# allenai/satlas-super-resolution

Hardware: AMD Instinct MI355X
Metric: G+D train-step images/sec (higher is better)
Workload: dtype fp32h

## Files before the change

satlas_super_resolution_amd/csrc/conv_x3r.hip:

```cpp
#include "conv_x3r_core.h"

#ifdef SSR_PROBE
#define RPROBE(cond, k) do { if (cond) g_probe[(blockIdx.y * gridDim.x + blockIdx.x) * 16 + (k)] = __builtin_amdgcn_s_memtime(); } while (0)
#else
#define RPROBE(cond, k)
#endif

namespace {

template <int NTW, int NU, int EP, int TH = 8, int AM = 0>
__global__ __launch_bounds__((XrT<NTW, NU, TH>::NTHR)) void conv_x3r_kernel(const ssr_conv_desc d) {
    constexpr bool EX = AM == 1, H = AM == 2;
    using T = XrT<NTW, NU, TH>;
    constexpr int NT = NTW, NTT = T::NTT, NMF = T::NMF, BN = T::BN, WR = T::WR, MT = T::MT;
    constexpr int G_NPIX = T::NPIX, G_SUB = T::SUB, G_PV = T::PV, G_NPV = T::NPV;
    extern __shared__ __attribute__((aligned(16))) char smem[];
    int* ctl = reinterpret_cast<int*>(smem + T::CTL);
    const int ctl_addr = (int)(size_t)(__attribute__((address_space(3))) char*)(smem + T::CTL);
    const int tid = threadIdx.x, lane = tid & 63, wave = __builtin_amdgcn_readfirstlane(tid >> 6);
    const int tiles_x = (d.Gw + 15) / 16, tiles_y = (d.Gh + TH - 1) / TH;
    int b = blockIdx.x;
    const int tx_i = b % tiles_x; b /= tiles_x;
    const int ty_i = b % tiles_y;
    const int n = b / tiles_y;
    const int gy0 = ty_i * TH, gx0 = tx_i * 16;
    const int co0 = blockIdx.y * BN;
    const int Cin = d.Cin, Cin2 = d.Cin2;
    const int nchunks = (Cin + Cin2 + 15) / 16;
    const int cout_pad = d.CoutPad;
    const int tapstride = cout_pad * 64, wchunk = 9 * tapstride;
    RPROBE(tid == 0, 0);
    if (tid < 4 + NMF) ctl[tid] = 0;
    __syncthreads();

    f32x16 acc[MT][NT];
#pragma unroll
    for (int t = 0; t < MT; ++t)
#pragma unroll
        for (int u = 0; u < NT; ++u)
#pragma unroll
            for (int r = 0; r < 16; ++r) acc[t][u][r] = 0.f;

    if (wave >= NMF) {
        const int pw = wave - NMF;
        const int pt = tid - 64 * NMF;
#ifdef XR_PRIO
        __builtin_amdgcn_s_setprio(3);
#endif
        const int part = pt & 3, p4 = pt >> 2;
        int ppix[G_NPV];
#pragma unroll
        for (int q = 0; q < G_NPV; ++q) {
            const int pix = p4 + 64 * q;
            const int py = pix / XR_PW, px = pix - py * XR_PW;
            const int ly = gy0 + py - d.pad_y, lx = gx0 + px - d.pad_x;
            const bool okp = pix < G_NPIX && ly >= 0 && ly < d.Hi && lx >= 0 && lx < d.Wi;
            ppix[q] = okp ? (n * d.Hi + ly) * d.Wi + lx : -1;
        }
        const int plo0 = p4 * XR_ROWB + part * 8;
        const long xbytes = (long)d.N * d.Hi * d.Wi * 4;
        const void* xp = d.x.p;
        const void* x2p = d.x2.p ? d.x2.p : d.x.p;
        const int x_cs = d.x.cs, x_coff = d.x.coff, x2_cs = d.x2.p ? d.x2.cs : d.x.cs, x2_coff = d.x2.p ? d.x2.coff : d.x.coff;
        u32x4 rq[XR_PQ][G_NPV];
        auto load_chunk = [&](int c, auto jc) {
            constexpr int j = decltype(jc)::value;
            const bool live = c < nchunks;
            const int c0 = c * 16;
            const bool in_x = c0 < Cin;
            const int cb = in_x ? c0 : c0 - Cin, clim = live ? (in_x ? Cin : Cin2) : 0;
            const int cs = in_x ? x_cs : x2_cs, coff = in_x ? x_coff : x2_coff;
            const __amdgpu_buffer_rsrc_t rs = xr_rsrc(in_x ? xp : x2p, xbytes * cs);
            const int k = cb + part * 4;
#pragma unroll
            for (int q = 0; q < G_NPV; ++q) {
                const int off = (ppix[q] * cs + coff + k) * 4;
                const bool okl = (k < clim) & (ppix[q] >= 0);
#ifdef XR_X_NOXLOAD
                rq[j][q] = u32x4{(unsigned)off, (unsigned)okl, 0u, 0u};
#else
                rq[j][q] = __builtin_amdgcn_raw_buffer_load_b128(rs, okl ? off : XR_OOB, 0, 0);
#endif
            }
        };
        static_for<0, XR_PQ>([&](auto jc) { __builtin_amdgcn_sched_barrier(0); load_chunk(decltype(jc)::value, jc); __builtin_amdgcn_sched_barrier(0); });
        RPROBE(pt == 0, 8);
        int cfree = XR_NS;
        for (int c0 = 0; c0 < nchunks; c0 += XR_PQ) {
            static_for<0, XR_PQ>([&](auto jc) {
                constexpr int j = decltype(jc)::value;
                const int c = c0 + j;
                if (c < nchunks) {
                    if (c >= cfree) {
                        int spin = 0;
                        for (; spin < XR_SPIN_MAX; ++spin) {
                            cfree = xr_minN<NMF>(ctl_addr + 16) + XR_NS;
                            if (c < cfree) break;
                            __builtin_amdgcn_s_sleep(2);
                        }
                        if (spin == XR_SPIN_MAX) __builtin_trap();
                    }
                    char* base = smem + (c % XR_NS) * G_SUB;
#pragma unroll
                    for (int q = 0; q < G_NPV; ++q) {
#ifdef XR_X_NOSTORE
                        asm volatile("" :: "v"(rq[j][q]));
                        continue;
#endif
                        if constexpr (EX) {
                            if (q < G_NPV - 1 || pt < G_PV - (G_NPV - 1) * 256)
                                *reinterpret_cast<u32x4*>(base + p4 * XR_ROWB + part * 16 + q * 64 * XR_ROWB) = rq[j][q];
                        } else {
                            uint2 hi, lo;
                            split_f32x4<H>(rq[j][q], hi, lo);
                            if (q < G_NPV - 1 || pt < G_PV - (G_NPV - 1) * 256) {
                                *reinterpret_cast<uint2*>(base + plo0 + q * 64 * XR_ROWB) = hi;
                                *reinterpret_cast<uint2*>(base + plo0 + q * 64 * XR_ROWB + 32) = lo;
                            }
                        }
                    }
                    asm volatile("" ::: "memory");
                    if (lane == 0) *(xr_lds_int)(uintptr_t)(ctl_addr + 4 * pw) = c + 1;
                    asm volatile("" ::: "memory");
#if defined(XR_PRIO) && XR_PRIO == 1
                    if (c == 0) __builtin_amdgcn_s_setprio(0);
#endif
                }
                __builtin_amdgcn_sched_barrier(0);
                load_chunk(c + XR_PQ, jc);
                __builtin_amdgcn_sched_barrier(0);
            });
        }
        RPROBE(pt == 0, 9);
    } else {
        const int w = wave & 3, ug = wave >> 2;
        const int i = lane & 31, gq = lane >> 5;
        const int a_lane = ((i >> 4) * XR_PW + epi_col<XR_ROT>(i)) * XR_ROWB + gq * 16;
        const __amdgpu_buffer_rsrc_t rsw = xr_rsrc(d.w, (long)nchunks * wchunk);
        const int w_lane = (co0 + 32 * NTW * ug + i) * 64 + gq * 16;
        const int nitems = 3 * nchunks;
        const int nj = nitems > w ? (nitems - w + 3) / 4 : 0;
        const int glast = w + 4 * (nj - 1);
        if (nj == 0) {
            if (lane == 0) *(xr_lds_int)(uintptr_t)(ctl_addr + 16 + 4 * wave) = 0x3fffffff;
        } else {
            bf16x8 wf[WR][NT][2];
            constexpr int TPS = T::TPS, SPT = T::SPT, NSUB = 3 * SPT, NSETS = T::NSETS, PD = NSETS - 1;
            bf16x8 af[NSETS][TPS][2];
            auto load_w = [&](int g_, auto kxc, auto sc) {
                constexpr int kx = decltype(kxc)::value, s = decltype(sc)::value;
                const int gg = g_ < glast ? g_ : glast;
                const int c = gg / 3, ky = gg - 3 * c;
                const int off = c * wchunk + (ky * 3 + kx) * tapstride + w_lane;
#pragma unroll
                for (int u = 0; u < NT; ++u) {
                    wf[s][u][0] = __builtin_bit_cast(bf16x8, __builtin_amdgcn_raw_buffer_load_b128(rsw, off + u * 2048, 0, 0));
                    wf[s][u][1] = __builtin_bit_cast(bf16x8, __builtin_amdgcn_raw_buffer_load_b128(rsw, off + u * 2048 + 32, 0, 0));
                }
            };
            auto issue_a = [&](int base, auto qc, auto sc, auto hc) {
                constexpr int q = decltype(qc)::value, kx = q / SPT, part = q % SPT, s = decltype(sc)::value, H = decltype(hc)::value;
#pragma unroll
                for (int t2 = 0; t2 < TPS; ++t2)
                    af[s][t2][H] = *reinterpret_cast<const bf16x8*>(smem + base + kx * XR_ROWB + (part * TPS + t2) * XR_TILEB + 32 * H);
            };
            int avail = 0;
            auto ensure = [&](int c) {
                if (avail > c) return;
                int spin = 0;
                for (; spin < XR_SPIN_MAX; ++spin) {
                    avail = xr_min4(ctl_addr);
                    if (avail > c) break;
                    __builtin_amdgcn_s_sleep(1);
                }
                if (spin == XR_SPIN_MAX) __builtin_trap();
            };
            auto base_of = [&](int g_) { const int c = g_ / 3, ky = g_ - 3 * c; return (c % XR_NS) * G_SUB + ky * XR_PW * XR_ROWB + a_lane; };
            using I0 = std::integral_constant<int, 0>;
            using I1 = std::integral_constant<int, 1>;
#ifndef XR_WPRE
#define XR_WPRE 99
#endif
            constexpr int WPRE = XR_WPRE < WR ? XR_WPRE : WR;
            static_for<0, WPRE>([&](auto sc) {
                constexpr int s = decltype(sc)::value;
                __builtin_amdgcn_sched_barrier(0);
                load_w(w + 4 * (s / 3), std::integral_constant<int, s % 3>{}, sc);
                __builtin_amdgcn_sched_barrier(0);
            });
            RPROBE(tid == 0, 1);
            int g = w, c_cur = g / 3;
            int base_cur = base_of(g);
            ensure(c_cur);
            static_for<WPRE, WR>([&](auto sc) {
                constexpr int s = decltype(sc)::value;
                __builtin_amdgcn_sched_barrier(0);
                load_w(w + 4 * (s / 3), std::integral_constant<int, s % 3>{}, sc);
                __builtin_amdgcn_sched_barrier(0);
            });
            RPROBE(tid == 0, 2);
            static_for<0, PD>([&](auto qc) {
                issue_a(base_cur, qc, std::integral_constant<int, decltype(qc)::value % NSETS>{}, I1{});
                issue_a(base_cur, qc, std::integral_constant<int, decltype(qc)::value % NSETS>{}, I0{});
            });
            int gn = g + 4 < glast ? g + 4 : glast;
            int c_next = gn / 3, base_next = base_of(gn);
            int gnn = gn, c_nn = c_next, base_nn = base_next;
            auto body = [&](int j, auto jpc) {
                constexpr int JP = decltype(jpc)::value;
                static_for<0, NSUB>([&](auto qc) {
                    constexpr int q = decltype(qc)::value, kx = q / SPT, part = q % SPT, qn = q + PD;
                    constexpr int ws = (JP * 3 + kx) % WR, as = (JP * NSUB + q) % NSETS, asn = (JP * NSUB + qn) % NSETS;
                    auto group = [&](auto pc) {
                        constexpr int P = decltype(pc)::value;
                        if constexpr (EX) {
                            constexpr int H = P == 0 ? 1 : 0, S0 = P == 2 ? 2 : 0, S1 = P == 1 ? 2 : 4;
#pragma unroll
                            for (int sidx = S0; sidx < S1; ++sidx)
#pragma unroll
                                for (int t2 = 0; t2 < TPS; ++t2)
#pragma unroll
                                    for (int u = 0; u < NT; ++u) {
                                        const f32x4 av = __builtin_bit_cast(f32x4, af[as][t2][H]), bv = __builtin_bit_cast(f32x4, wf[ws][u][H]);
                                        acc[part * TPS + t2][u] = __builtin_amdgcn_mfma_f32_32x32x2f32(av[sidx], bv[sidx], acc[part * TPS + t2][u], 0, 0, 0);
                                    }
                        } else {
#pragma unroll
                            for (int t2 = 0; t2 < TPS; ++t2)
#pragma unroll
                                for (int u = 0; u < NT; ++u)
                                    acc[part * TPS + t2][u] = split_mfma<H>(af[as][t2][P == 0 ? 1 : 0], wf[ws][u][P == 1 ? 1 : 0], acc[part * TPS + t2][u]);
                        }
                    };
                    auto reads = [&](auto hc) {
#ifndef XR_X_NOA
                        if constexpr (qn < NSUB) issue_a(base_cur, std::integral_constant<int, qn>{}, std::integral_constant<int, asn>{}, hc);
                        else issue_a(base_next, std::integral_constant<int, qn - NSUB>{}, std::integral_constant<int, asn>{}, hc);
#endif
                    };
                    __builtin_amdgcn_sched_barrier(0);
                    if constexpr (qn == NSUB) {
                        if (c_next > c_cur) {
                            asm volatile("" ::: "memory");
                            if (lane == 0) *(xr_lds_int)(uintptr_t)(ctl_addr + 16 + 4 * wave) = c_next;
                            asm volatile("" ::: "memory");
                        }
                        ensure(c_next);
                        __builtin_amdgcn_sched_barrier(0);
                    }
                    group(std::integral_constant<int, 0>{});
                    __builtin_amdgcn_sched_barrier(0);
                    reads(I1{});
                    if constexpr (part == 0) {
#ifndef XR_X_NOW
                        constexpr int wsp = (JP * 3 + kx + WR - 1) % WR, ioff = (kx + WR - 1) / 3, tap = (kx + WR - 1) % 3;
                        load_w(g + 4 * ioff, std::integral_constant<int, tap>{}, std::integral_constant<int, wsp>{});
#endif
                    }
                    __builtin_amdgcn_sched_barrier(0);
                    group(std::integral_constant<int, 1>{});
                    __builtin_amdgcn_sched_barrier(0);
                    reads(I0{});
                    if constexpr (q == 0) {
                        gnn = g + 8 < glast ? g + 8 : glast;
                        c_nn = gnn / 3;
                        base_nn = base_of(gnn);
                    }
                    __builtin_amdgcn_sched_barrier(0);
                    group(std::integral_constant<int, 2>{});
                    __builtin_amdgcn_sched_barrier(0);
                });
                g += 4;
                c_cur = c_next; base_cur = base_next;
                gn = gnn; c_next = c_nn; base_next = base_nn;
#ifdef SSR_PROBE
                if (j < 5) RPROBE(tid == 0, 3 + j);
#endif
            };
            if constexpr (WR == 6 || (NSUB % NSETS) != 0) {
                for (int j = 0; j < nj; j += 2) {
                    body(j, std::integral_constant<int, 0>{});
                    if (j + 1 < nj) body(j + 1, std::integral_constant<int, 1>{});
                }
            } else {
                for (int j = 0; j < nj; ++j) body(j, std::integral_constant<int, 0>{});
            }
            asm volatile("" ::: "memory");
            if (lane == 0) *(xr_lds_int)(uintptr_t)(ctl_addr + 16 + 4 * wave) = 0x3fffffff;
        }
    }
    __syncthreads();
    RPROBE(tid == 0, 10);

    const bool is_mfma = wave < NMF;
    const int me = is_mfma ? (wave & 3) : wave - NMF;
    const int ut = is_mfma ? NTW * (wave >> 2) : 1;
#ifndef XR_X_NORED
    if (is_mfma) {
#pragma unroll
        for (int t = 0; t < MT; ++t)
#pragma unroll
            for (int u = 0; u < NT; ++u)
                if (!(t == me && u == 0)) {
                    char* sp = smem + ((me * MT + t) * NTT + ut + u) * XR_SLOT + lane * 16;
#pragma unroll
                    for (int q = 0; q < 4; ++q) {
                        f32x4 v = {acc[t][u][4 * q], acc[t][u][4 * q + 1], acc[t][u][4 * q + 2], acc[t][u][4 * q + 3]};
                        *reinterpret_cast<f32x4*>(sp + q * 1024) = v;
                    }
                }
    }
#endif
    __syncthreads();
    if ((is_mfma || NTW == 2) && me < MT) {
        f32x16 own;
#pragma unroll
        for (int r = 0; r < 16; ++r) own[r] = 0.f;
        if (is_mfma) {
#pragma unroll
            for (int t = 0; t < MT; ++t)
                if (t == me) own = acc[t][0];
        }
        f32x16 sum;
#pragma unroll
        for (int s = 0; s < 4; ++s) {
            f32x16 part;
            const char* sp = smem + ((s * MT + me) * NTT + ut) * XR_SLOT + lane * 16;
#ifdef XR_X_NORED
            part = own;
            asm volatile("" : "+v"(part));
#else
#pragma unroll
            for (int q = 0; q < 4; ++q) {
                const f32x4 v = *reinterpret_cast<const f32x4*>(sp + q * 1024);
                part[4 * q] = v[0]; part[4 * q + 1] = v[1]; part[4 * q + 2] = v[2]; part[4 * q + 3] = v[3];
            }
#endif
            const bool mine = is_mfma && s == me;
#pragma unroll
            for (int r = 0; r < 16; ++r) {
                const float p = mine ? own[r] : part[r];
                sum[r] = s == 0 ? p : sum[r] + p;
            }
        }
        if constexpr (H) {
#pragma unroll
            for (int r = 0; r < 16; ++r) sum[r] *= SSR_F32H_UNSCALE;
        }
        char* slab = smem + (((is_mfma ? me : 0) * MT + me) * NTT + ut) * XR_SLOT;
        const int cb = co0 + 32 * ut;
#ifdef XR_X_NOEPI
        float keep = 0.f;
#pragma unroll
        for (int r = 0; r < 16; ++r) keep += sum[r];
        if (keep == 123.456f) reinterpret_cast<float*>(d.y.p)[tid] = keep;
#else
        if constexpr (EP == XR_EP_GENERIC) conv_epilogue<float, XR_ROT>(d, sum, cb, n, gy0 + 2 * me, gx0, lane, slab);
        else xr_epilogue<EP>(d, sum, cb, n, gy0 + 2 * me, gx0, lane, slab);
#endif
    }
    RPROBE(tid == 0, 11);
}

template <int NTW, int NU, int EP, int TH = 8, int AM = 0>
int launch_x3r(const ssr_conv_desc& d, hipStream_t st) {
    using T = XrT<NTW, NU, TH>;
    auto kern = conv_x3r_kernel<NTW, NU, EP, TH, AM>;
    static bool attr_done[SSR_MAX_DEVICES] = {};
    const int dev = ssr_device_ordinal();
    if (!attr_done[dev]) {
        hipError_t e = hipFuncSetAttribute(reinterpret_cast<const void*>(kern), hipFuncAttributeMaxDynamicSharedMemorySize, T::LDS);
        if (e != hipSuccess) return (int)e;
        attr_done[dev] = true;
    }
    const int tiles = ((d.Gw + 15) / 16) * ((d.Gh + TH - 1) / TH) * d.N;
    hipLaunchKernelGGL(kern, dim3(tiles, d.CoutPad / T::BN, 1), dim3(T::NTHR), T::LDS, st, d);
    SSR_LAUNCH_CHECK();
    return SSR_OK;
}

int xr_pick_epilogue(const ssr_conv_desc& d) {
    static const bool generic_only = [] { const char* e = getenv("SSR_X3R_EPI"); return e && e[0] == '0'; }();
    if (generic_only) return XR_EP_GENERIC;
    const long lim = 0x7fffff00L, npx = (long)d.N * d.Ho * d.Wo * 4;
    auto vok = [&](const ssr_view& v) { return (v.cs % 4) == 0 && (v.coff % 4) == 0 && ((uintptr_t)v.p % 16) == 0 && npx * v.cs <= lim; };
    if (d.fix_list || d.y0.p || d.y1.p || d.accumulate || d.m_relu || (d.Cout % 4) != 0 || !vok(d.y)) return XR_EP_GENERIC;
    if (d.oys != 1 || d.oxs != 1 || d.oyo != 0 || d.oxo != 0 || d.Ho < d.Gh || d.Wo < d.Gw) return XR_EP_GENERIC;
    const bool r1 = d.r1.p != nullptr, r2 = d.r2.p != nullptr, m = d.m.p != nullptr;
    if (d.act == SSR_ACT_LRELU && d.alpha == 1.f && !r1 && !r2 && !m) return XR_EP_LRELU;
    if (d.act == SSR_ACT_NONE && !m && (!r1 || (d.r1_nc >= d.Cout && vok(d.r1))) && (!r2 || (d.r2_nc >= d.Cout && vok(d.r2)))) return XR_EP_LIN;
    if (d.act == SSR_ACT_NONE && d.alpha == 1.f && m && !r1 && !r2 && d.m_c0 == 0 && d.m_c1 >= d.Cout && vok(d.m)) return XR_EP_MASK;
    return XR_EP_GENERIC;
}

template <int NTW, int NU, int TH = 8, int AM = 0>
int launch_x3r_ep(const ssr_conv_desc& d, hipStream_t st) {
    switch (xr_pick_epilogue(d)) {
        case XR_EP_LRELU: return launch_x3r<NTW, NU, XR_EP_LRELU, TH, AM>(d, st);
        case XR_EP_LIN: return launch_x3r<NTW, NU, XR_EP_LIN, TH, AM>(d, st);
        case XR_EP_MASK: return launch_x3r<NTW, NU, XR_EP_MASK, TH, AM>(d, st);
        default: return launch_x3r<NTW, NU, XR_EP_GENERIC, TH, AM>(d, st);
    }
}

int xr_tile_height(const ssr_conv_desc& d, int form) {
    static const int forced = [] { const char* e = getenv("SSR_X3_REGTILE_TH"); return e ? atoi(e) : 0; }();
    if (form != 0) return 8;
    if (forced == 4 || forced == 8) return forced;
    const long tiles8 = (long)((d.Gw + 15) / 16) * ((d.Gh + 7) / 8) * d.N * (d.CoutPad / 32);
    return (tiles8 <= 160 && d.Gh > 4) ? 4 : 8;
}

int xr_wide_form(const ssr_conv_desc& d) {
    static const int f = [] { const char* e = getenv("SSR_X3_REGTILE_NT2"); return !e ? 1 : e[0] == '0' ? 0 : e[0] == '8' ? 2 : 1; }();
    if ((d.CoutPad % 64) != 0) return 0;
    static const bool split_off = [] { const char* e = getenv("SSR_X3_REGTILE_SPLIT"); return e && e[0] == '0'; }();
    const long tiles = (long)((d.Gw + 15) / 16) * ((d.Gh + 7) / 8) * d.N;
    if (!split_off && tiles * (d.CoutPad / 64) <= 160) return 0;
    return (f == 2 && xr_pick_epilogue(d) == XR_EP_GENERIC) ? 1 : f;
}

}

void ssr_conv_x3r_instance(const ssr_conv_desc& d, int* ntw, int* nu, int* ep) {
    int f = xr_wide_form(d);
    if ((d.dtype == SSR_F32 || d.dtype == SSR_F32H) && f == 2) f = 1;
    *ntw = f == 1 ? 2 : 1;
    *nu = f == 2 ? 2 : 1;
    *ep = xr_pick_epilogue(d);
}
int ssr_conv_x3r_tile_height(const ssr_conv_desc& d) { return xr_tile_height(d, xr_wide_form(d)); }

bool ssr_conv_x3r_shape_ok(const ssr_conv_desc& d) {
    static const bool ex_off = [] { const char* e = getenv("SSR_F32_REGTILE"); return e && e[0] == '0'; }();
    if (!(d.dtype == SSR_F32X3 || d.dtype == SSR_F32H || (d.dtype == SSR_F32 && !ex_off)) || d.fix_list) return false;
    if (d.dtype == SSR_F32 && (d.act == SSR_ACT_RELU || d.m_relu)) return false;
    if (!(d.KH == 3 && d.KW == 3 && d.stride == 1 && d.pad_y == 1 && d.pad_x == 1 && d.up == 1 && !d.s2d)) return false;
    if (d.Gh != d.Hi || d.Gw != d.Wi || (d.CoutPad % 32) != 0) return false;
    if (d.x2.p && (d.Cin % 16) != 0) return false;
    const long lim = 0x7fffff00L, npx = (long)d.N * d.Hi * d.Wi * 4;
    if (npx * d.x.cs > lim || (d.x2.p && npx * d.x2.cs > lim)) return false;
    if ((long)((d.Cin + d.Cin2 + 15) / 16) * 9 * d.CoutPad * 64 > lim) return false;
    return true;
}

bool ssr_conv_x3r_qualifies(const ssr_conv_desc& d) {
    static const bool off = [] { const char* e = getenv("SSR_X3_REGTILE"); return e && e[0] == '0'; }();
    if (off || !ssr_conv_x3r_shape_ok(d)) return false;
    return d.Gh <= 64 && d.Gw <= 64 && d.Cin + d.Cin2 >= 16;
}

bool ssr_conv_x3r_try(const ssr_conv_desc& d, hipStream_t st, int* rc, bool force) {
    if (force ? !ssr_conv_x3r_shape_ok(d) : !ssr_conv_x3r_qualifies(d)) return false;
    const int f = xr_wide_form(d);
    if (d.dtype == SSR_F32) {
        if (f != 0) *rc = launch_x3r_ep<2, 1, 8, 1>(d, st);
        else *rc = xr_tile_height(d, f) == 4 ? launch_x3r_ep<1, 1, 4, 1>(d, st) : launch_x3r_ep<1, 1, 8, 1>(d, st);
        return true;
    }
    if (d.dtype == SSR_F32H) {
        if (f != 0) *rc = launch_x3r_ep<2, 1, 8, 2>(d, st);
        else *rc = xr_tile_height(d, f) == 4 ? launch_x3r_ep<1, 1, 4, 2>(d, st) : launch_x3r_ep<1, 1, 8, 2>(d, st);
        return true;
    }
    if (f == 2) *rc = launch_x3r_ep<1, 2>(d, st);
    else if (f == 1) *rc = launch_x3r_ep<2, 1>(d, st);
    else *rc = xr_tile_height(d, f) == 4 ? launch_x3r_ep<1, 1, 4>(d, st) : launch_x3r_ep<1, 1, 8>(d, st);
    return true;
}
```

Before: 1194.

## Replace syncthreads with raw LDS barriers and simplify cross-wave accumulator reduction

Swaps __syncthreads for a hand-written s_waitcnt lgkmcnt(0)+s_barrier. The initial barrier now sits after each role issues its first global prefetches, so those loads are in flight across it. The reduction now writes every accumulator tile to LDS, own tile included, and reads all four partials back. This drops the per-register select logic and the live 'own' copy, at the cost of extra LDS traffic. It also pins descriptor fields to scalar registers and adds placement/realtime probes that compile only under SSR_PROBE.

```diff
diff --git a/satlas_super_resolution_amd/csrc/conv_x3r.hip b/satlas_super_resolution_amd/csrc/conv_x3r.hip
--- a/satlas_super_resolution_amd/csrc/conv_x3r.hip
+++ b/satlas_super_resolution_amd/csrc/conv_x3r.hip
@@ -2,8 +2,15 @@
 
 #ifdef SSR_PROBE
 #define RPROBE(cond, k) do { if (cond) g_probe[(blockIdx.y * gridDim.x + blockIdx.x) * 16 + (k)] = __builtin_amdgcn_s_memtime(); } while (0)
+#define RPROBE_WHERE(cond, k) do { if (cond) { unsigned hw_, xcc_; asm volatile("s_getreg_b32 %0, hwreg(HW_REG_HW_ID)" : "=s"(hw_)); \
+    asm volatile("s_getreg_b32 %0, hwreg(HW_REG_XCC_ID)" : "=s"(xcc_)); \
+    g_probe[(blockIdx.y * gridDim.x + blockIdx.x) * 16 + 12] = ((unsigned long long)xcc_ << 32) | hw_; \
+    g_probe[(blockIdx.y * gridDim.x + blockIdx.x) * 16 + (k)] = __builtin_amdgcn_s_memrealtime(); } } while (0)
+#define RPROBE_REAL(cond, k) do { if (cond) g_probe[(blockIdx.y * gridDim.x + blockIdx.x) * 16 + (k)] = __builtin_amdgcn_s_memrealtime(); } while (0)
 #else
 #define RPROBE(cond, k)
+#define RPROBE_WHERE(cond, k)
+#define RPROBE_REAL(cond, k)
 #endif
 
 namespace {
@@ -18,6 +25,8 @@
     int* ctl = reinterpret_cast<int*>(smem + T::CTL);
     const int ctl_addr = (int)(size_t)(__attribute__((address_space(3))) char*)(smem + T::CTL);
     const int tid = threadIdx.x, lane = tid & 63, wave = __builtin_amdgcn_readfirstlane(tid >> 6);
+    asm volatile("" :: "s"(d.Gw), "s"(d.Gh), "s"(d.Cin), "s"(d.Cin2), "s"(d.CoutPad), "s"(d.w), "s"(d.x.p), "s"(d.x.cs), "s"(d.x.coff),
+                 "s"(d.x2.p), "s"(d.x2.cs), "s"(d.x2.coff), "s"(d.N), "s"(d.Hi), "s"(d.Wi), "s"(d.pad_y), "s"(d.pad_x));
     const int tiles_x = (d.Gw + 15) / 16, tiles_y = (d.Gh + TH - 1) / TH;
     int b = blockIdx.x;
     const int tx_i = b % tiles_x; b /= tiles_x;
@@ -29,9 +38,13 @@
     const int nchunks = (Cin + Cin2 + 15) / 16;
     const int cout_pad = d.CoutPad;
     const int tapstride = cout_pad * 64, wchunk = 9 * tapstride;
+    const void* const wp = d.w;
+    const void* const xp = d.x.p;
+    const void* const x2p = d.x2.p ? d.x2.p : d.x.p;
     RPROBE(tid == 0, 0);
+    RPROBE_WHERE(tid == 0, 14);
     if (tid < 4 + NMF) ctl[tid] = 0;
-    __syncthreads();
+    auto lds_barrier = [] { asm volatile("s_waitcnt lgkmcnt(0)\n\ts_barrier" ::: "memory"); };
 
     f32x16 acc[MT][NT];
 #pragma unroll
@@ -59,8 +72,6 @@
         }
         const int plo0 = p4 * XR_ROWB + part * 8;
         const long xbytes = (long)d.N * d.Hi * d.Wi * 4;
-        const void* xp = d.x.p;
-        const void* x2p = d.x2.p ? d.x2.p : d.x.p;
         const int x_cs = d.x.cs, x_coff = d.x.coff, x2_cs = d.x2.p ? d.x2.cs : d.x.cs, x2_coff = d.x2.p ? d.x2.coff : d.x.coff;
         u32x4 rq[XR_PQ][G_NPV];
         auto load_chunk = [&](int c, auto jc) {
@@ -84,6 +95,7 @@
             }
         };
         static_for<0, XR_PQ>([&](auto jc) { __builtin_amdgcn_sched_barrier(0); load_chunk(decltype(jc)::value, jc); __builtin_amdgcn_sched_barrier(0); });
+        lds_barrier();
         RPROBE(pt == 0, 8);
         int cfree = XR_NS;
         for (int c0 = 0; c0 < nchunks; c0 += XR_PQ) {
@@ -136,12 +148,13 @@
         const int w = wave & 3, ug = wave >> 2;
         const int i = lane & 31, gq = lane >> 5;
         const int a_lane = ((i >> 4) * XR_PW + epi_col<XR_ROT>(i)) * XR_ROWB + gq * 16;
-        const __amdgpu_buffer_rsrc_t rsw = xr_rsrc(d.w, (long)nchunks * wchunk);
+        const __amdgpu_buffer_rsrc_t rsw = xr_rsrc(wp, (long)nchunks * wchunk);
         const int w_lane = (co0 + 32 * NTW * ug + i) * 64 + gq * 16;
         const int nitems = 3 * nchunks;
         const int nj = nitems > w ? (nitems - w + 3) / 4 : 0;
         const int glast = w + 4 * (nj - 1);
         if (nj == 0) {
+            lds_barrier();
             if (lane == 0) *(xr_lds_int)(uintptr_t)(ctl_addr + 16 + 4 * wave) = 0x3fffffff;
         } else {
             bf16x8 wf[WR][NT][2];
@@ -188,6 +201,7 @@
                 load_w(w + 4 * (s / 3), std::integral_constant<int, s % 3>{}, sc);
                 __builtin_amdgcn_sched_barrier(0);
             });
+            lds_barrier();
             RPROBE(tid == 0, 1);
             int g = w, c_cur = g / 3;
             int base_cur = base_of(g);
@@ -289,45 +303,37 @@
             if (lane == 0) *(xr_lds_int)(uintptr_t)(ctl_addr + 16 + 4 * wave) = 0x3fffffff;
         }
     }
-    __syncthreads();
-    RPROBE(tid == 0, 10);
-
     const bool is_mfma = wave < NMF;
     const int me = is_mfma ? (wave & 3) : wave - NMF;
     const int ut = is_mfma ? NTW * (wave >> 2) : 1;
+    const bool finisher = (is_mfma || NTW == 2) && me < MT;
+    lds_barrier();
+    RPROBE(tid == 0, 10);
+
 #ifndef XR_X_NORED
     if (is_mfma) {
 #pragma unroll
         for (int t = 0; t < MT; ++t)
 #pragma unroll
-            for (int u = 0; u < NT; ++u)
-                if (!(t == me && u == 0)) {
-                    char* sp = smem + ((me * MT + t) * NTT + ut + u) * XR_SLOT + lane * 16;
-#pragma unroll
-                    for (int q = 0; q < 4; ++q) {
-                        f32x4 v = {acc[t][u][4 * q], acc[t][u][4 * q + 1], acc[t][u][4 * q + 2], acc[t][u][4 * q + 3]};
-                        *reinterpret_cast<f32x4*>(sp + q * 1024) = v;
-                    }
+            for (int u = 0; u < NT; ++u) {
+                char* sp = smem + ((me * MT + t) * NTT + ut + u) * XR_SLOT + lane * 16;
+#pragma unroll
+                for (int q = 0; q < 4; ++q) {
+                    f32x4 v = {acc[t][u][4 * q], acc[t][u][4 * q + 1], acc[t][u][4 * q + 2], acc[t][u][4 * q + 3]};
+                    *reinterpret_cast<f32x4*>(sp + q * 1024) = v;
                 }
-    }
-#endif
-    __syncthreads();
-    if ((is_mfma || NTW == 2) && me < MT) {
-        f32x16 own;
-#pragma unroll
-        for (int r = 0; r < 16; ++r) own[r] = 0.f;
-        if (is_mfma) {
-#pragma unroll
-            for (int t = 0; t < MT; ++t)
-                if (t == me) own = acc[t][0];
-        }
+            }
+    }
+#endif
+    lds_barrier();
+    if (finisher) {
         f32x16 sum;
 #pragma unroll
         for (int s = 0; s < 4; ++s) {
             f32x16 part;
             const char* sp = smem + ((s * MT + me) * NTT + ut) * XR_SLOT + lane * 16;
 #ifdef XR_X_NORED
-            part = own;
+            part = acc[0][0];
             asm volatile("" : "+v"(part));
 #else
 #pragma unroll
@@ -336,12 +342,8 @@
                 part[4 * q] = v[0]; part[4 * q + 1] = v[1]; part[4 * q + 2] = v[2]; part[4 * q + 3] = v[3];
             }
 #endif
-            const bool mine = is_mfma && s == me;
-#pragma unroll
-            for (int r = 0; r < 16; ++r) {
-                const float p = mine ? own[r] : part[r];
-                sum[r] = s == 0 ? p : sum[r] + p;
-            }
+#pragma unroll
+            for (int r = 0; r < 16; ++r) sum[r] = s == 0 ? part[r] : sum[r] + part[r];
         }
         if constexpr (H) {
 #pragma unroll
@@ -360,6 +362,7 @@
 #endif
     }
     RPROBE(tid == 0, 11);
+    RPROBE_REAL(tid == 0, 15);
 }
 
 template <int NTW, int NU, int EP, int TH = 8, int AM = 0>
```

Result: faster. 1208, median of 6 (+1.2%).
